# khanhha/multiview_motion_capture

Measured on AMD Instinct MI355X. Metric: frames/s (assoc+triangulate+IK) at C=5,P=4,J=25, higher is better.
Workload: dtype f64

## Files before the change

### include/mvmc.h

```cpp
#ifndef MVMC_H
#define MVMC_H

#include <stdint.h>

#ifdef __cplusplus
extern "C" {
#endif

#define MVMC_ABI_VERSION 6

enum {
    MVMC_OK = 0,
    MVMC_ERR_ARG = 1,
    MVMC_ERR_LAUNCH = 2,
    MVMC_ERR_UNSUPPORTED = 3
};

enum { MVMC_F32 = 0, MVMC_F64 = 1 };

#define MVMC_N_COCO 17
#define MVMC_N_SKEL 18
#define MVMC_N_SIDE 11
#define MVMC_N_PARAM 68
#define MVMC_MAX_NODES 80
// ... 160 lines not shown
    int32_t* out_meta;
    int32_t* out_n_tracks;
    double* out_info;
    int32_t* out_als_iters;
    uint32_t* flags;
    double* out_phase_cycles;
} mvmcChainBuffers;
int mvmc_chain_run(const mvmcSkeleton* skel_host, const mvmcChainBuffers* buffers, mvmcStream_t stream);

int mvmc_chain_run_rigs(const mvmcSkeleton* skel_host, const mvmcChainBuffers* buffers, const int32_t* rig_of_chain, int n_rigs,
                        mvmcStream_t stream);

int mvmc_chain_run_sessions(const mvmcSkeleton* skel_host, const mvmcChainBuffers* buffers, const int32_t* rig_of_chain, int n_rigs,
                            const uint8_t* active, mvmcStream_t stream);


int mvmc_body_observe(const double* kps17, const int32_t* counts, int n_frames, int n_views, int p_max, const double* Pmats,
                      int n_rigs, const int32_t* frame_of, const int32_t* rig_of, const double* joints, const int32_t* order,
                      const int32_t* grp_lo, const int32_t* grp_hi, const int32_t* rank, int n_problems, double min_score,
                      double max_dist, int32_t* choice, double* dist, int32_t* members, int32_t* n_views_out, mvmcStream_t stream);

#define MVMC_BODY_INFO_DOUBLES 16
#define MVMC_BODY_WORK_DOUBLES 270
int mvmc_body_lengths(const mvmcSkeleton* skel_host, const double* kps17, int n_views, int p_max, const double* Pmats,
                      const int32_t* rig_of, const int32_t* members, const double* params, const int32_t* id_lo, int n_ids,
                      double* lens, int32_t* free_mask, int fix_free, int max_iter, double mu0, double ftol, double xtol,
                      double* info, double* work, mvmcStream_t stream);

int mvmc_ik_solve_stages_rigs(const mvmcSkeleton* skel_host, const double* kps17, const double* Pmats, int n_rigs,
                              const int32_t* rig_of_problem, const int32_t* members, int n_problems, int v_max, int n_views,
// ... 115 lines not shown
```

### multiview_motion_capture_amd/_cabi.py

```python
from __future__ import annotations

import ctypes as C
import os

_LIB_PATH = os.environ.get("MVMC_LIB_PATH") or os.path.join(os.path.dirname(os.path.abspath(__file__)), "lib",
                                                           "libmvmc_hip.so")
_lib = None

MVMC_OK = 0
MVMC_ABI = 6
MVMC_F32, MVMC_F64 = 0, 1
N_PARAM = 68
MAX_NODES = 80
IK_SCRATCH_DOUBLES = 7680
IK_FD_WORK_DOUBLES = 40960
IK_STEP_OUT_DOUBLES = 240
BOUND_WORDS, ROW_WORDS = 56, 128
BODY_INFO_DOUBLES, BODY_WORK_DOUBLES = 16, 270
SMOOTH_K, SMOOTH_BLOCK_DOUBLES, SMOOTH_WORK_DOUBLES, SMOOTH_INFO_DOUBLES, SMOOTH_MAX_VIEWS = 39, 820, 3940, 32, 64
SMOOTH_COV_INFO_DOUBLES, SMOOTH_JOINTS = 8, 18
SMOOTH_WIN_MAX, SMOOTH_WIN_RING, SMOOTH_WIN_ITEM_INTS, SMOOTH_WIN_INFO_DOUBLES = 32, 66, 8, 16
RELINK_MAX_RECORDS, RELINK_REC_DOUBLES = 512, 120
RIG_TILE, RIG_MAX_CAMS, RIG_MAX_ITER, RIG_CAM_DOUBLES, RIG_INFO_DOUBLES = 64, 8, 24, 21, 64
LENS_DOUBLES, LENS_PINHOLE, LENS_BROWN, LENS_FISHEYE, LENS_MAX_ITER, LENS_FISHEYE_MAX_THETA = 16, 0, 1, 2, 12, 1.5
# ... 1 lines not shown
RIG_LOSS_NONE, RIG_LOSS_HUBER, RIG_LOSS_CAUCHY = 0, 1, 2
RIG_STOP = {0: "running", 1: "xtol", 2: "ftol", 3: "few_cameras", 4: "few_points", 5: "max_iter"}

SYMBOLS = (
    "mvmc_abi_version", "mvmc_status_string", "mvmc_als_seed_table", "mvmc_ingest", "mvmc_fmats",
    "mvmc_affinity", "mvmc_als_associate", "mvmc_closure_labels", "mvmc_cluster_members", "mvmc_dlt", "mvmc_triangulate_postopt", "mvmc_fk", "mvmc_ik_solve",
    "mvmc_fmats_from_projections", "mvmc_st_affinity", "mvmc_track_assign", "mvmc_track_commit", "mvmc_debug_eigh",
    "mvmc_debug_trstep", "mvmc_ik_solve_stages", "mvmc_chain_run", "mvmc_svt_associate", "mvmc_debug_ik_solve_fd", "mvmc_debug_ik_model_step", "mvmc_ingest_dlt", "mvmc_ingest_dlt_f32", "mvmc_pack_message_words", "mvmc_pack_work_words", "mvmc_stitch_work_words", "mvmc_pack_tracks", "mvmc_stitch_chains",
    "mvmc_chain_run_rigs", "mvmc_chain_run_sessions", "mvmc_body_observe", "mvmc_body_lengths", "mvmc_ik_solve_stages_rigs",
    "mvmc_smooth_blocks", "mvmc_smooth_step", "mvmc_smooth_cov", "mvmc_smooth_window_work_doubles", "mvmc_smooth_window", "mvmc_relink_work_words", "mvmc_relink",
    "mvmc_rig_part_doubles", "mvmc_rig_red_doubles", "mvmc_rig_start", "mvmc_rig_accumulate", "mvmc_rig_step",
    "mvmc_rig_accumulate_robust", "mvmc_rig_step_robust", "mvmc_rig_weights",
    "mvmc_rig_part_doubles_intr", "mvmc_rig_red_doubles_intr", "mvmc_rig_accumulate_intr", "mvmc_rig_step_intr",
    "mvmc_lens_undistort", "mvmc_lens_distort",
    "mvmc_pair_moments", "mvmc_pair_consensus", "mvmc_pair_refit",
)


class MvmcSkeleton(C.Structure):
    _fields_ = [("bone_dirs", (C.c_double * 3) * 18), ("parents", C.c_int32 * 18),
                ("side_map", C.c_int32 * 18), ("n_side", C.c_int32), ("ref_side_lens", C.c_double * 18)]


class MvmcChainBuffers(C.Structure):
    _INTS = ("n_chains", "chain_len", "n_views", "p_max", "t_max", "k_max", "v_max", "max_nfev_cold", "max_nfev_warm",
             "n_inits", "seed_len", "n_parts", "force_big", "hand_over")
    _PTRS = ("kps17", "counts", "Pmats", "Fmats", "F2", "seed_table", "params", "joints", "meta", "n_tracks", "next_id",
             "n_dead", "slot_src", "S_sp", "W_st", "group_counts", "labels_sp", "labels_st", "n_clusters_sp", "n_clusters_st",
             "iters_sp", "iters_st", "members", "n_members", "cold", "init", "status", "n_new", "ik_params", "ik_joints", "ik_info",
             "ik_scratch", "out_params", "out_joints", "out_meta", "out_n_tracks", "out_info", "out_als_iters", "flags", "out_phase_cycles")
    _fields_ = [(n, C.c_int32) for n in _INTS] + [(n, C.c_void_p) for n in _PTRS]


class MvmcError(RuntimeError):
    pass


def lib_path() -> str:
    return _LIB_PATH


def build_info():
    if os.environ.get("MVMC_LIB_PATH"):
        return None
    from . import _buildinfo
    return _buildinfo.read()
# ... 37 lines not shown
        "mvmc_dlt": [vp, vp, vp, i32, i32, i32, i32, i32, f64, vp, vp],
        "mvmc_ingest_dlt": [vp, i32, i32, i32, i32, i32, vp, f64, i32, f64, vp, vp, i32, i32, f64, vp, vp, vp],
        "mvmc_ingest_dlt_f32": [vp, i32, i32, i32, i32, vp, f64, i32, f64, vp, vp, i32, i32, f64, vp, vp, vp],
        "mvmc_triangulate_postopt": [vp, vp, vp, i32, i32, i32, i32, i32, vp, vp],
        "mvmc_fk": [SK, vp, i32, vp, vp, vp],
        "mvmc_ik_solve": [SK, vp, vp, vp, i32, i32, i32, i32, vp, vp, i32, i32, vp, vp, vp, vp, vp],
        "mvmc_fmats_from_projections": [vp, i32, vp, vp],
        "mvmc_st_affinity": [vp, vp, vp, vp, vp, vp, vp, i32, i32, i32, i32, f64, vp, vp, vp, vp],
        "mvmc_track_assign": [vp] * 8 + [i32] * 6 + [vp] * 7,
        "mvmc_track_commit": [vp] * 4 + [i32] * 4 + [vp] * 9,
        "mvmc_debug_eigh": [vp, vp, i32, i32, vp, vp, vp, vp, vp],
        "mvmc_debug_trstep": [vp, vp, i32, i32, i32, f64, f64, vp, vp, vp, vp],
        "mvmc_chain_run": [SK, C.POINTER(MvmcChainBuffers), vp],
        "mvmc_chain_run_rigs": [SK, C.POINTER(MvmcChainBuffers), vp, i32, vp],
        "mvmc_chain_run_sessions": [SK, C.POINTER(MvmcChainBuffers), vp, i32, vp, vp],
        "mvmc_ik_solve_stages": [SK, vp, vp, vp, vp, i32, i32, i32, i32, vp, i32, i32, vp, vp, vp, vp, vp],
        "mvmc_debug_ik_solve_fd": [SK, vp, vp, vp, i32, i32, i32, i32, vp, vp, i32, i32, i32, vp, vp, vp, vp, vp],
        "mvmc_debug_ik_model_step": [SK, vp, vp, vp, i32, i32, i32, i32, vp, i32, vp, vp, vp, vp, vp],
        "mvmc_pack_message_words": [i32, i32, i32, i32],
        "mvmc_pack_work_words": [i32, i32, i32],
        "mvmc_stitch_work_words": [i32, i32, i32],
        "mvmc_pack_tracks": [vp, vp, vp, vp, vp, i32, i32, i32, i32, i32, i32, i32, f64, vp, i32, vp, vp, vp],
        "mvmc_stitch_chains": [vp, C.c_longlong, i32, i32, i32, i32, i32, f64, i32, vp, vp, vp, vp, vp],
        "mvmc_body_observe": [vp, vp, i32, i32, i32, vp, i32, vp, vp, vp, vp, vp, vp, vp, i32, f64, f64, vp, vp, vp, vp, vp],
        "mvmc_body_lengths": [SK, vp, i32, i32, vp, vp, vp, vp, vp, i32, vp, vp, i32, i32, f64, f64, f64, vp, vp, vp],
        "mvmc_ik_solve_stages_rigs": [SK, vp, vp, i32, vp, vp, i32, i32, i32, i32, vp, i32, i32, vp, vp, vp, vp, vp],
        "mvmc_smooth_blocks": [SK, vp, i32, i32, vp, vp, vp, vp, vp, vp, i32, vp, vp],
        "mvmc_smooth_step": [SK, vp, vp, vp, vp, i32, i32, f64, f64, f64, f64, f64, f64, f64, i32, i32, vp, vp, vp, vp],
        "mvmc_smooth_cov": [SK, vp, vp, vp, i32, i32, f64, f64, f64, f64, f64, vp, i32, i32, vp, vp, vp, vp, vp, vp, vp, vp],
        "mvmc_smooth_window_work_doubles": [i32, i32],
# ... 46 lines not shown
```

### multiview_motion_capture_amd/csrc/mvmc_assoc.hip

```cpp
#if !defined(MVMC_DEVICE_ONLY) && !defined(MVMC_SMALL_WPS)
#define MVMC_SMALL_WPS 4
#define ALS4_WG_PER_CU 4
#endif
#include "mvmc_common.h"

namespace {

template <typename T>
__global__ void __launch_bounds__(256)
ingest_kernel(const T* __restrict__ kps, int C, int P, int J_in, const int32_t* __restrict__ counts_in,
              double min_score, int min_valid, double min_bb, double* __restrict__ kps17,
              int32_t* __restrict__ counts_out) {
    extern __shared__ double sm[];
    const int f = blockIdx.x;
    const int nq = C * P;
    double* pose = sm;
    int* keep = reinterpret_cast<int*>(sm + nq * 51);
    int* src_of = keep + nq;
    const T* src = kps + (size_t)f * nq * J_in * 3;
    for (int e = threadIdx.x; e < nq * 51; e += blockDim.x) {
        int q = e / 51, r = e - q * 51, j = r / 3, k = r - j * 3;
        int js = (J_in == 25) ? op25_to_coco17(j) : j;
        pose[e] = (double)src[(q * J_in + js) * 3 + k];
    }
    __syncthreads();
    for (int q = threadIdx.x; q < nq; q += blockDim.x) {
        int c = q / P, p = q - c * P;
        int cnt = counts_in ? counts_in[f * C + c] : P;
        int ok = 0;
        if (p < cnt) {
            int nv = 0;
            double x0 = 1e300, x1 = -1e300, y0 = 1e300, y1 = -1e300;
            for (int j = 0; j < 17; ++j) {
                const double* kp = pose + q * 51 + j * 3;
                if (kp[2] > min_score) {
                    ++nv;
                    x0 = fmin(x0, kp[0]); x1 = fmax(x1, kp[0]);
                    y0 = fmin(y0, kp[1]); y1 = fmax(y1, kp[1]);
                }
            }
            ok = (nv >= min_valid) && !((x1 - x0) < min_bb || (y1 - y0) < min_bb);
        }
        keep[q] = ok;
    }
    __syncthreads();
    for (int c = threadIdx.x; c < C; c += blockDim.x) {
        int k = 0;
        for (int p = 0; p < P; ++p)
            if (keep[c * P + p]) src_of[c * P + k++] = c * P + p;
        counts_out[f * C + c] = k;
        for (; k < P; ++k) src_of[c * P + k] = -1;
    }
    __syncthreads();
    double* out = kps17 + (size_t)f * nq * 51;
    for (int e = threadIdx.x; e < nq * 51; e += blockDim.x) {
        int d = e / 51, r = e - d * 51;
        int q = src_of[d];
        out[e] = q >= 0 ? pose[q * 51 + r] : 0.0;
    }
}

__device__ inline void m3mul(const double* A, const double* B, double* O) {
    for (int i = 0; i < 3; ++i)
        for (int j = 0; j < 3; ++j) {
            double s = 0;
            for (int k = 0; k < 3; ++k) s += A[i * 3 + k] * B[k * 3 + j];
            O[i * 3 + j] = s;
        }
}
__device__ inline void m3t(const double* A, double* O) {
    for (int i = 0; i < 3; ++i)
        for (int j = 0; j < 3; ++j) O[i * 3 + j] = A[j * 3 + i];
}
__device__ inline void m3v(const double* A, const double* x, double* o) {
// ... 1799 lines not shown
        }
    }
}

}

#ifndef MVMC_DEVICE_ONLY
extern "C" int mvmc_ingest(const void* kps, int dtype, int n_frames, int n_views, int p_max, int n_joints_in,
                           const int32_t* counts_in, double min_score, int min_valid, double min_bb_size,
                           double* kps17, int32_t* counts_out, mvmcStream_t stream) {
    if (!kps || !kps17 || !counts_out || n_frames < 0 || n_views <= 0 || p_max <= 0) return MVMC_ERR_ARG;
    if (n_joints_in != 25 && n_joints_in != 17) return MVMC_ERR_ARG;
    if (dtype != MVMC_F32 && dtype != MVMC_F64) return MVMC_ERR_ARG;
    if (n_frames == 0) return MVMC_OK;
    const int nq = n_views * p_max;
    size_t shm = (size_t)nq * 51 * sizeof(double) + (size_t)nq * 2 * sizeof(int);
    if (shm > 64 * 1024) return MVMC_ERR_UNSUPPORTED;
    hipStream_t s = (hipStream_t)stream;
    if (dtype == MVMC_F32)
        hipLaunchKernelGGL(ingest_kernel<float>, dim3(n_frames), dim3(256), shm, s, (const float*)kps, n_views, p_max,
                           n_joints_in, counts_in, min_score, min_valid, min_bb_size, kps17, counts_out);
    else
        hipLaunchKernelGGL(ingest_kernel<double>, dim3(n_frames), dim3(256), shm, s, (const double*)kps, n_views,
                           p_max, n_joints_in, counts_in, min_score, min_valid, min_bb_size, kps17, counts_out);
    MVMC_CHECK_LAUNCH();
    return MVMC_OK;
}

extern "C" int mvmc_fmats(const double* K, const double* Rt, int n_views, float* F, mvmcStream_t stream) {
    if (!K || !Rt || !F || n_views <= 0) return MVMC_ERR_ARG;
    int n = n_views * n_views;
// ... 84 lines not shown
```

### multiview_motion_capture_amd/csrc/mvmc_chain.hip

```cpp
#define MVMC_DEVICE_ONLY
#if !defined(MVMC_CHAIN_BIG_TU) && !defined(MVMC_SMALL_WPS)
#define MVMC_SMALL_WPS 4
#endif
#if !defined(MVMC_CHAIN_BIG_TU) && !defined(MVMC_PRIO_ALS) && !defined(MVMC_NO_PHASE_PRIO)
#define MVMC_PRIO_ALS 1
#define MVMC_PRIO_REST 1
#endif
#if defined(MVMC_WITH_IK_PAIR) && !defined(MVMC_CHAIN_BIG_TU) && !defined(MVMC_CHAIN_LAT_TU) && MVMC_SMALL_WPS >= 4
#define MVMC_IK_PAIR 1
#endif
#include <cstdlib>
#include "mvmc_common.h"
#include "mvmc_assoc.hip"
#include "mvmc_track.hip"
#include "mvmc_ik1.hip"

struct MvmcChainArgs {
    const double* kps17;
    const int32_t* counts;
    const double* Pm;
    const float* Fm;
    const double* F2;
    const double* seed;
    int seed_len;
// ... 26 lines not shown
    double* ik_scratch;
    double* out_params;
    double* out_joints;
    int32_t* out_meta;
    int32_t* out_n;
    double* out_info;
    int32_t* out_iters;
    double* out_cycles;
    int parts;
    int queue;
    unsigned* flags;
    int self_zero;
    const int32_t* rig;
    int n_rigs;
    const uint8_t* active;
};


namespace {

using ChainArgs = MvmcChainArgs;
using ChainArgsK = const __attribute__((address_space(4))) MvmcChainArgs;

struct ChainRig { const double* Pm; const float* Fm; const double* F2; bool ok; };
__device__ __forceinline__ ChainRig chain_rig(ChainArgsK& A, int b) {
    ChainRig g{A.Pm, A.Fm, A.F2, true};
    if (A.rig) {
        const int r = uni(mvmc_ld_i32(A.rig + b));
        g.ok = r >= 0 && r < A.n_rigs;
        if (g.ok && r > 0) {
// ... 60 lines not shown
        if (2 * 4 * P * 68 <= CH_KOFF_BIG && C * P <= 64) {
            st_pose_pairs_lines<ChainCfg<BIG>::NT>(arena.graph + CH_EOFF_BIG, arena.graph, kf, A.counts, f, F2, C, P, 0.1);
            Epre = arena.graph + CH_EOFF_BIG;
        }
    }
    st_affinity_wave<ChainCfg<BIG>::NT>(arena.graph, A.kps17, A.counts, 0, f, A.joints + (size_t)b * T * 54, A.n_tracks + b, Pm, F2, C, P,
                           T, 0.1, W, nullptr, A.gc + (size_t)b * (C + 1), Epre, C * P, kf);
    *done = 0;
}
__device__ __noinline__ void chain_pose_pairs(ChainArena<false>& arena_in, ChainArgsK& A, int f, const double* F2_in, int* done) {
    ChainArena<false>& arena = *uni(&arena_in);
    MVMC_ASSUME_LDS(&arena);
    st_pose_pairs(arena.graph + CH_EOFF, A.kps17, A.counts, f, uni(F2_in), A.C, A.P, 0.1);
    *done = 0;
}
template <bool BIG>
__device__ __noinline__ void chain_als_spatial(ChainArena<BIG>& arena_in, ChainArgsK& A, int b, int f, int* done) {
    ChainArena<BIG>& arena = *uni(&arena_in);
    MVMC_ASSUME_LDS(&arena);
    const int C = A.C, N = C * A.P;
    if constexpr (BIG)
        als5_graph<float, 72>(arena.als, 0, A.S_sp + (size_t)b * N * N, A.counts + (size_t)f * C, C, N, A.seed, A.seed_len,
                                          nullptr, nullptr, A.labels_sp + (size_t)b * N, A.ncl_sp + b, A.iters_sp + b);
    else
        als4_graph<float, 24>(arena.als_sp, 0, A.S_sp + (size_t)b * N * N, A.counts + (size_t)f * C, C, N, A.seed, A.seed_len, nullptr,
                              nullptr, A.labels_sp + (size_t)b * N, A.ncl_sp + b, A.iters_sp + b);
    *done = 0;
}
template <bool BIG>
__device__ __noinline__ void chain_als_temporal(ChainArena<BIG>& arena_in, ChainArgsK& A, int b, int* done) {
// ... 96 lines not shown
    }
    {
        static_assert(sizeof(Ik1Tables) % 4 == 0, "copied by words");
        typedef const __attribute__((address_space(4))) unsigned* KernargWords;
        KernargWords src = (KernargWords)__builtin_amdgcn_kernarg_segment_ptr();
        unsigned* dst = reinterpret_cast<unsigned*>(&tables);
        for (int i = tid; i < (int)(sizeof(Ik1Tables) / 4); i += ChainCfg<BIG>::NT) dst[i] = src[i];
    }
    int b, part;
    int done = 0;
    ChainRig rig{A.Pm, A.Fm, A.F2, true};
    if (!queue) {
        const int idx = by_ticket ? uni(s_nt) : (int)blockIdx.x;
        b = idx % A.n_chains; part = idx / A.n_chains;
        rig = chain_rig(A, b);
        if constexpr (!BIG) { if (part > 0 && rig.ok) chain_pose_pairs(arena, A, b * A.L + part * A.L / A.parts, rig.F2, &done); }
    }
    if (queue || part > 0) {
        if (tid == 0) {
            int task = queue ? (int)ticket : ((part << 20) | b);
            const bool must_wait = queue ? ticket >= (unsigned)A.n_chains : true;
            if (must_wait) {
                const unsigned* word = queue ? qwords + 2 + (ticket - (unsigned)A.n_chains) : A.flags + b;
                const unsigned need = queue ? 1u : (unsigned)part;
                const unsigned long long t0 = wall_clock64();
                bool abort = false;
                unsigned spins = 0, v;
                while ((v = __hip_atomic_load(word, __ATOMIC_RELAXED, __HIP_MEMORY_SCOPE_AGENT)) < need) {
                    __builtin_amdgcn_s_sleep(32);
                    if ((++spins & 1023u) != 0u) continue;
// ... 8 lines not shown
                asm volatile("s_waitcnt vmcnt(0)" ::: "memory");
                if (queue && !abort) task = (int)v - 1;
                if (abort) {
                    if (!queue) __hip_atomic_store(A.flags + b, (unsigned)(part + 1), __ATOMIC_RELAXED, __HIP_MEMORY_SCOPE_AGENT);
                    task = -1;
                }
            }
            s_task = task;
        }
        __syncthreads();
        const int task = uni(s_task);
        if (task < 0) return;
        b = task & 0xFFFFF; part = task >> 20;
        if (queue) {
            rig = chain_rig(A, b);
            if constexpr (!BIG) { if (part > 0 && rig.ok) chain_pose_pairs(arena, A, b * A.L + part * A.L / A.parts, rig.F2, &done); }
        }
    }
    if (A.active && uni((int)A.active[b]) == 0) return;
    const int T = A.T, NP = T + A.K;
    const int t_lo = part * A.L / A.parts;
    int t_hi = (part + 1) * A.L / A.parts;
    if (!rig.ok) {
        for (int t = t_lo + tid; t < t_hi; t += ChainCfg<BIG>::NT) A.out_n[b * A.L + t] = 0;
        if (tid == 0) atomicOr(A.flags + A.n_chains + 4 + b, 16u);
        t_hi = t_lo;
    }
    __syncthreads();
    long long cyc[6] = {0, 0, 0, 0, 0, 0}, t_prev = clock64();
    const long long t_start = t_prev;
    auto lap = [&](int k) { const long long now = clock64(); cyc[k] += now - t_prev; t_prev = now; };
    for (int t = t_lo; t < t_hi; ++t) {
        const int f = b * A.L + t;
        if (tid == 0) s_nt = mvmc_ld_i32(A.n_tracks + b);
        __syncthreads();
        const int nt = uni(s_nt);
#ifdef MVMC_PRIO_ALS
        if constexpr (!BIG) __builtin_amdgcn_s_setprio(MVMC_PRIO_ALS);
#endif
        if (nt <= 0) {
            chain_graph_spatial<BIG>(arena, A, b, f, rig.Fm, &done);
            __syncthreads();
            lap(0);
            chain_als_spatial<BIG>(arena, A, b, f, &done);
        } else {
            chain_graph_temporal<BIG>(arena, A, b, f, part > 0 && t == t_lo, rig.Pm, rig.F2, &done);
            __syncthreads();
            lap(0);
// ... 87 lines not shown
    MVMC_CHECK_LAUNCH();
    return MVMC_OK;
}
#else
extern "C" int mvmc_chain_run(const mvmcSkeleton* skel_host, const mvmcChainBuffers* buf, mvmcStream_t stream) {
    return mvmc_chain_run_rigs(skel_host, buf, nullptr, 1, stream);
}

extern "C" int mvmc_chain_run_rigs(const mvmcSkeleton* skel_host, const mvmcChainBuffers* buf, const int32_t* rig_of_chain, int n_rigs,
                                   mvmcStream_t stream) {
    return mvmc_chain_run_sessions(skel_host, buf, rig_of_chain, n_rigs, nullptr, stream);
}

extern "C" int mvmc_chain_run_sessions(const mvmcSkeleton* skel_host, const mvmcChainBuffers* buf, const int32_t* rig_of_chain, int n_rigs,
                                       const uint8_t* active, mvmcStream_t stream) {
    if (!skel_host || !buf) return MVMC_ERR_ARG;
    if (n_rigs < 1 || (!rig_of_chain && n_rigs != 1)) return MVMC_ERR_ARG;
    const mvmcChainBuffers& B = *buf;
    if (active && B.n_parts > 1) return MVMC_ERR_ARG;
    if (B.n_chains < 0 || B.chain_len <= 0 || B.n_views <= 0 || B.p_max <= 0 || B.t_max <= 0 || B.k_max <= 0 || B.v_max <= 0)
        return MVMC_ERR_ARG;
    if (B.max_nfev_cold < 1 || B.max_nfev_warm < 1) return MVMC_ERR_ARG;
    const int N = B.n_views * B.p_max, NS = B.t_max + N;
    if (B.n_views > 16 || 2 * B.p_max > 16) return MVMC_ERR_UNSUPPORTED;
    if (B.t_max + B.k_max > 64 || B.v_max > 64) return MVMC_ERR_UNSUPPORTED;
    const bool small = N <= ChainCfg<false>::N_MAX && NS <= ChainCfg<false>::NS_MAX && !B.force_big &&
                       2 * (B.t_max > B.p_max ? B.t_max : B.p_max) <= 16;
    const bool big = N <= ChainCfg<true>::N_MAX && NS <= ChainCfg<true>::NS_MAX && B.t_max <= 16;
    if (!small && !big) return MVMC_ERR_UNSUPPORTED;
    const void* need[] = {B.kps17, B.counts, B.Pmats, B.Fmats, B.F2, B.seed_table, B.params, B.joints, B.meta, B.n_tracks,
                          B.next_id, B.n_dead, B.slot_src, B.S_sp, B.W_st, B.group_counts, B.labels_sp, B.labels_st, B.n_clusters_sp,
// ... 15 lines not shown
    A.S_sp = B.S_sp; A.W_st = B.W_st; A.gc = B.group_counts; A.labels_sp = B.labels_sp; A.labels_st = B.labels_st;
    A.ncl_sp = B.n_clusters_sp; A.ncl_st = B.n_clusters_st; A.iters_sp = B.iters_sp; A.iters_st = B.iters_st;
    A.members = B.members; A.n_members = B.n_members; A.cold = B.cold; A.init = B.init; A.status = B.status;
    A.n_new = B.n_new; A.ik_params = B.ik_params; A.ik_joints = B.ik_joints; A.ik_info = B.ik_info; A.ik_scratch = B.ik_scratch;
    A.out_params = B.out_params; A.out_joints = B.out_joints; A.out_meta = B.out_meta; A.out_n = B.out_n_tracks;
    A.out_info = B.out_info; A.out_iters = B.out_als_iters; A.out_cycles = B.out_phase_cycles;
    A.parts = B.n_parts > 1 ? B.n_parts : 1;
    if (A.parts > 1 && B.chain_len % A.parts != 0) return MVMC_ERR_ARG;
    if (B.hand_over < 0 || B.hand_over > 2) return MVMC_ERR_ARG;
    A.queue = B.hand_over;
    if (B.n_chains >= (1 << 20) || A.parts >= (1 << 10)) return MVMC_ERR_UNSUPPORTED;
    A.flags = B.flags;
    A.self_zero = 0;
    A.rig = rig_of_chain; A.n_rigs = n_rigs;
    A.active = active;
    bool lat = false;
    if (small) {
        static const bool no_lat = getenv("MVMC_CHAIN_NO_LAT") && atoi(getenv("MVMC_CHAIN_NO_LAT")) != 0;
        int dev = 0, cus = 256;
        if (hipGetDevice(&dev) == hipSuccess) {
            int v = 0;
            if (hipDeviceGetAttribute(&v, hipDeviceAttributeMultiprocessorCount, dev) == hipSuccess && v > 0) cus = v;
        }
        lat = !no_lat && (long long)B.n_chains * A.parts <= 2LL * cus;
    }
    if (lat && B.n_chains == 1 && A.parts == 1)
        A.self_zero = 1;
    else if (hipMemsetAsync(B.flags, 0, sizeof(unsigned) * ((size_t)B.n_chains * (A.parts + 1) + 8), (hipStream_t)stream) != hipSuccess)
        return MVMC_ERR_LAUNCH;
    Ik1Tables tables_host;
// ... 16 lines not shown
```

### multiview_motion_capture_amd/pipeline.py

```python
from __future__ import annotations

from typing import Optional

import torch

from . import device as dev


class HotPath:
    def __init__(self, K, Rt, device="cuda:0", k_max: Optional[int] = None, v_max: Optional[int] = None):
        d = torch.device(device)
        self.device = d
        self.K = torch.as_tensor(K, dtype=torch.float64, device=d).contiguous()
        self.Rt = torch.as_tensor(Rt, dtype=torch.float64, device=d).contiguous()
        self.P = torch.bmm(self.K, self.Rt).contiguous()
        self.F = dev.fmats(self.K, self.Rt)
        self.skeleton = dev.make_skeleton()
        self.k_max = k_max
        self.v_max = v_max

    def associate(self, kps: torch.Tensor, counts: Optional[torch.Tensor] = None, want_mats=False):
        kps17, cnt = dev.ingest(kps, counts)
        P = kps17.shape[2]
        D, S = dev.affinity(kps17, cnt, self.F, want_D=want_mats)
        res = dev.als_associate(S, cnt, g_max=P, want_mats=want_mats)
        res.update(kps17=kps17, counts=cnt, D=D, S=S)
        return res

    def triangulate(self, assoc: dict):
        kps17, cnt = assoc["kps17"], assoc["counts"]
        C, P = kps17.shape[1], kps17.shape[2]
        k_max = self.k_max or max(1, (C * P) // 2)
        v_max = self.v_max or min(C * P, 64)
        mem, nm = dev.cluster_members(assoc["labels"], cnt, P, k_max, v_max)
# ... 19 lines not shown
```

### multiview_motion_capture_amd/tracker.py

```python
from __future__ import annotations

import ctypes
import os
from typing import Optional, Sequence

import numpy as np
import torch

from . import _cabi, device as dev
from .pipeline import HotPath

T_WIDE = 16


class ChainFlags:
    CLUSTER, TRACKS, GRAPH, IK_PAIR, RIG = 1, 2, 4, 8, 16
    REPAIRABLE = CLUSTER | TRACKS | GRAPH

    def __init__(self, words, n_chains: int):
        B = n_chains
        self.words, self.B, self._v0 = words, B, B + 4

    @staticmethod
    def length(n_chains: int, n_parts: int) -> int:
# ... 28 lines not shown
                                 (F.TRACKS, "more than t_max live tracklets")) if bits & bit]
        return ValueError(f"{who}: capacity exceeded (" + "; ".join(what) + f") in {n_void} chain(s): their results are void")
    return None


def _verdict_of(timeout, void: np.ndarray, who: str) -> Optional[Exception]:
    return void_verdict(int(timeout), int(np.bitwise_or.reduce(void)), int(np.count_nonzero(void)), who)


def _raise_if_void(timeout, void: np.ndarray, who: str) -> None:
    exc = _verdict_of(timeout, void, who)
    if exc is not None:
        raise exc


def chain_workspace(B: int, n_out: int, C: int, P: int, T: int, K: int, V: int, d, want_info: bool, flags) -> dict:
    N, NS, NP = C * P, T + C * P, T + K
    f64, i32 = torch.float64, torch.int32
    e = lambda shape, dt: torch.empty(shape, dtype=dt, device=d)
    z = lambda shape, dt: torch.zeros(shape, dtype=dt, device=d)
    return dict(
        seed_table=dev.als_seed_table(_cabi.MAX_NODES * _cabi.MAX_NODES, d),
        S_sp=e((B, N, N), torch.float32), W_st=e((B, NS, NS), f64), group_counts=e((B, C + 1), i32),
        labels_sp=e((B, N), i32), labels_st=e((B, NS), i32), n_clusters_sp=z((B,), i32), n_clusters_st=z((B,), i32),
        iters_sp=z((B,), i32), iters_st=z((B,), i32), members=e((B, NP, V), i32), n_members=z((B, NP), i32),
        cold=e((B, NP), torch.uint8), init=e((B, NP, 68), f64), status=e((B, T), i32), n_new=e((B,), i32),
        ik_params=e((B, NP, 68), f64), ik_joints=e((B, NP, 18, 3), f64), ik_info=e((B, NP, 8), f64),
        ik_scratch=dev.stream_buffer("chain_ik", B, (8, _cabi.IK_SCRATCH_DOUBLES), d),
        out_params=e((n_out, T, 68), f64), out_joints=e((n_out, T, 18, 3), f64), out_meta=e((n_out, T, 4), i32),
        out_n_tracks=e((n_out,), i32), out_info=e((n_out, NP, 8), f64) if want_info else None,
        out_als_iters=e((n_out,), i32) if want_info else None, out_phase_cycles=e((B, 8), f64) if want_info else None,
        flags=z((flags,), i32) if isinstance(flags, int) else flags)


def fill_chain_buffers(ints: dict, tensors: dict) -> "_cabi.MvmcChainBuffers":
    buf = _cabi.MvmcChainBuffers()
    odd = (set(ints) ^ set(buf._INTS)) | (set(tensors) ^ set(buf._PTRS))
    if odd:
        raise ValueError(f"a chain buffer is not named or not known: {sorted(odd)}")
    for name in buf._INTS:
        setattr(buf, name, int(ints[name]))
    for name in buf._PTRS:
        setattr(buf, name, None if tensors[name] is None else tensors[name].data_ptr())
    return buf


def launch_chain(skeleton, buf, d, rig_of_chain: Optional[torch.Tensor] = None, n_rigs: int = 1,
                 active: Optional[torch.Tensor] = None) -> None:
    lib, sk, bf = _cabi.load(), ctypes.byref(skeleton), ctypes.byref(buf)
    stream = ctypes.c_void_p(torch.cuda.current_stream(d).cuda_stream)
    rig = None if rig_of_chain is None else ctypes.c_void_p(rig_of_chain.data_ptr())
    if active is not None:
        _cabi.check(lib.mvmc_chain_run_sessions(sk, bf, rig, n_rigs, ctypes.c_void_p(active.data_ptr()), stream), "mvmc_chain_run_sessions")
    elif rig is not None:
        _cabi.check(lib.mvmc_chain_run_rigs(sk, bf, rig, n_rigs, stream), "mvmc_chain_run_rigs")
    else:
        _cabi.check(lib.mvmc_chain_run(sk, bf, stream), "mvmc_chain_run")


def default_caps(n_views: int, p_max: int):
    n = n_views * p_max
    return max(1, n // 2), min(n, 64)


class ChainTracker:
    def __init__(self, hp: HotPath, n_chains: int, p_max: int, t_max: int = 8, k_max: Optional[int] = None,
                 v_max: Optional[int] = None, nfev_cold=50, nfev_warm=5, rigs: Optional[Sequence[HotPath]] = None):
# ... 334 lines not shown
    if rigs is None and rig_of_chain is not None:
        raise ValueError("run_chains_fused: rig_of_chain needs rigs")
    roc = None if rigs is None else check_rig_of_chain(rig_of_chain, B, len(rigs))
    if parts is None:
        parts = L
    if parts > 1 and L % parts:
        raise ValueError("run_chains_fused: parts must divide the chain length")
    if hand_over is None:
        hand_over = "ticket"
    if hand_over not in ("static", "queue", "ticket"):
        raise ValueError("run_chains_fused: hand_over must be 'ticket', 'static' or 'queue'")
    T = t_max if t_max is not None else (T_WIDE if Cn * P > 40 else 8)
    k_def, v_def = default_caps(Cn, P)
    K = k_max or k_def
    V = v_max or v_def
    kps17, cnt = dev.ingest(kps, counts)
    d = kps.device
    if rigs is None:
        Pm, Fm, F2 = hp.P, hp.F, dev.fmats_from_projections(hp.P)
    else:
        Pm, Fm, F2 = stack_rigs(rigs, Cn)
    f64, i32 = torch.float64, torch.int32
    z = lambda shape, dt: torch.zeros(shape, dtype=dt, device=d)
    t = dict(chain_workspace(B, F, Cn, P, T, K, V, d, want_info, ChainFlags.length(B, parts)),
             kps17=kps17, counts=cnt, Pmats=Pm, Fmats=Fm, F2=F2,
             params=z((B, T, 68), f64), joints=z((B, T, 18, 3), f64), meta=z((B, T, 4), i32), n_tracks=z((B,), i32),
             next_id=z((B,), i32), n_dead=z((B,), i32), slot_src=torch.full((B, T), -1, dtype=i32, device=d))
    ints = dict(n_chains=B, chain_len=L, n_views=Cn, p_max=P, t_max=T, k_max=K, v_max=V, max_nfev_cold=nfev_cold,
                max_nfev_warm=nfev_warm, n_inits=3, seed_len=t["seed_table"].numel(), n_parts=parts, force_big=int(force_big),
                hand_over={"static": 0, "queue": 1, "ticket": 2}[hand_over])
    buf = fill_chain_buffers(ints, t)
    rig_dev = None if roc is None else torch.from_numpy(roc).to(d)
    if kernel_events is not None:
        k0, k1 = torch.cuda.Event(enable_timing=True), torch.cuda.Event(enable_timing=True)
        k0.record()
    launch_chain(hp.skeleton, buf, d, rig_dev, 1 if rigs is None else len(rigs))
    if kernel_events is not None:
        k1.record()
        kernel_events.append((k0, k1))
    fl = ChainFlags(t["flags"], B)
    res = dict(params=t["out_params"], joints=t["out_joints"], meta=t["out_meta"], n_tracks=t["out_n_tracks"],
               n_dead=t["n_dead"], next_id=t["next_id"], flags=t["flags"], void=fl.void, void_words=fl.status, n_chains=B,
               chain_len=L, _keepalive=dict(t, rig_of_chain=rig_dev))
    if rigs is not None:
        res["rigs"], res["rig_of_chain"] = list(rigs), roc
    if want_info:
        res["ik_info"] = t["out_info"].view(B, L, T + K, 8)
        res["als_iters"] = t["out_als_iters"].view(B, L)
        res["phase_cycles"] = t["out_phase_cycles"]
    return res

# ... 13 lines not shown
    if a.size and not np.issubdtype(a.dtype, np.integer):
        raise ValueError(f"rig_of_chain: integer indices, not {a.dtype}")
    if a.size and (a.min() < 0 or a.max() >= n_rigs):
        raise ValueError(f"rig_of_chain: indices in [{a.min()}, {a.max()}], the call has {n_rigs} rig(s)")
    return np.ascontiguousarray(a, dtype=np.int32)


def stack_rigs(rigs: Sequence[HotPath], n_views: int):
    if len(rigs) == 0:
        raise ValueError("rigs: at least one rig")
    for r, h in enumerate(rigs):
        if h.P.shape[0] != n_views:
            raise ValueError(f"rigs[{r}] has {h.P.shape[0]} cameras, the keypoints {n_views} views")
    Pm = torch.stack([h.P for h in rigs]).contiguous()
    Fm = torch.stack([h.F for h in rigs]).contiguous()
    F2 = torch.stack([dev.fmats_from_projections(h.P) for h in rigs]).contiguous()
    return Pm, Fm, F2


def check_chain_flags(res) -> None:
    if "flags" not in res:
        _raise_if_void(0, res["overflow"].cpu().numpy(), "run_chains")
        return
    fl = ChainFlags(res["flags"], res["n_chains"]).host()
    _raise_if_void(fl.timeout, fl.void, "mvmc_chain_run")


def repair_chains(hp: HotPath, kps: torch.Tensor, counts: Optional[torch.Tensor], res, nfev_cold=50, nfev_warm=5,
                  t_wide: int = T_WIDE, big_first: bool = True) -> int:
    B, L = res["n_chains"], res["chain_len"]
    fl = ChainFlags(res["flags"], B)
# ... 72 lines not shown
```

Baseline: 563,100.

## Fuse keypoint ingest and state init into the chain kernel

Moves the per-frame keypoint ingest (joint remap, validity filter, compaction) into the persistent chain kernel, which stages each frame in LDS scratch and publishes it with a release/acquire fence. Per-chain track state is now zeroed on the device, so the separate ingest launch and the host-side torch.zeros/full allocations are replaced by empty tensors. It also caches F2 per hot path so it is no longer recomputed on every call. This cuts launch and memset overhead at the cost of extra in-kernel syncs and ingest work on the critical path.

New measurement: 564,400 (median of 6 runs). Within noise of the previous version (+0.2%).

```diff
diff --git a/include/mvmc.h b/include/mvmc.h
--- a/include/mvmc.h
+++ b/include/mvmc.h
@@ -198,6 +198,20 @@
 int mvmc_chain_run_sessions(const mvmcSkeleton* skel_host, const mvmcChainBuffers* buffers, const int32_t* rig_of_chain, int n_rigs,
                             const uint8_t* active, mvmcStream_t stream);
 
+typedef struct mvmcChainFront {
+    const void* kps_raw;
+    int32_t kps_dtype;
+    int32_t n_joints_in;
+    const int32_t* counts_in;
+    double ingest_min_score;
+    int32_t min_valid;
+    double min_bb_size;
+    int32_t fresh_state;
+} mvmcChainFront;
+
+int mvmc_chain_run_front(const mvmcSkeleton* skel_host, const mvmcChainBuffers* buffers, const mvmcChainFront* front,
+                         const int32_t* rig_of_chain, int n_rigs, const uint8_t* active, mvmcStream_t stream);
+
 
 int mvmc_body_observe(const double* kps17, const int32_t* counts, int n_frames, int n_views, int p_max, const double* Pmats,
                       int n_rigs, const int32_t* frame_of, const int32_t* rig_of, const double* joints, const int32_t* order,
diff --git a/multiview_motion_capture_amd/_cabi.py b/multiview_motion_capture_amd/_cabi.py
--- a/multiview_motion_capture_amd/_cabi.py
+++ b/multiview_motion_capture_amd/_cabi.py
@@ -39,6 +39,7 @@
     "mvmc_rig_part_doubles_intr", "mvmc_rig_red_doubles_intr", "mvmc_rig_accumulate_intr", "mvmc_rig_step_intr",
     "mvmc_lens_undistort", "mvmc_lens_distort",
     "mvmc_pair_moments", "mvmc_pair_consensus", "mvmc_pair_refit",
+    "mvmc_chain_run_front",
 )
 
 
@@ -55,6 +56,11 @@
              "iters_sp", "iters_st", "members", "n_members", "cold", "init", "status", "n_new", "ik_params", "ik_joints", "ik_info",
              "ik_scratch", "out_params", "out_joints", "out_meta", "out_n_tracks", "out_info", "out_als_iters", "flags", "out_phase_cycles")
     _fields_ = [(n, C.c_int32) for n in _INTS] + [(n, C.c_void_p) for n in _PTRS]
+
+
+class MvmcChainFront(C.Structure):
+    _fields_ = [("kps_raw", C.c_void_p), ("kps_dtype", C.c_int32), ("n_joints_in", C.c_int32), ("counts_in", C.c_void_p),
+                ("ingest_min_score", C.c_double), ("min_valid", C.c_int32), ("min_bb_size", C.c_double), ("fresh_state", C.c_int32)]
 
 
 class MvmcError(RuntimeError):
@@ -122,6 +128,7 @@
         "mvmc_chain_run": [SK, C.POINTER(MvmcChainBuffers), vp],
         "mvmc_chain_run_rigs": [SK, C.POINTER(MvmcChainBuffers), vp, i32, vp],
         "mvmc_chain_run_sessions": [SK, C.POINTER(MvmcChainBuffers), vp, i32, vp, vp],
+        "mvmc_chain_run_front": [SK, C.POINTER(MvmcChainBuffers), C.POINTER(MvmcChainFront), vp, i32, vp, vp],
         "mvmc_ik_solve_stages": [SK, vp, vp, vp, vp, i32, i32, i32, i32, vp, i32, i32, vp, vp, vp, vp, vp],
         "mvmc_debug_ik_solve_fd": [SK, vp, vp, vp, i32, i32, i32, i32, vp, vp, i32, i32, i32, vp, vp, vp, vp, vp],
         "mvmc_debug_ik_model_step": [SK, vp, vp, vp, i32, i32, i32, i32, vp, i32, vp, vp, vp, vp, vp],
diff --git a/multiview_motion_capture_amd/csrc/mvmc_assoc.hip b/multiview_motion_capture_amd/csrc/mvmc_assoc.hip
--- a/multiview_motion_capture_amd/csrc/mvmc_assoc.hip
+++ b/multiview_motion_capture_amd/csrc/mvmc_assoc.hip
@@ -3,6 +3,7 @@
 #define ALS4_WG_PER_CU 4
 #endif
 #include "mvmc_common.h"
+#include "mvmc_ingest.h"
 
 namespace {
 
@@ -12,52 +13,7 @@
               double min_score, int min_valid, double min_bb, double* __restrict__ kps17,
               int32_t* __restrict__ counts_out) {
     extern __shared__ double sm[];
-    const int f = blockIdx.x;
-    const int nq = C * P;
-    double* pose = sm;
-    int* keep = reinterpret_cast<int*>(sm + nq * 51);
-    int* src_of = keep + nq;
-    const T* src = kps + (size_t)f * nq * J_in * 3;
-    for (int e = threadIdx.x; e < nq * 51; e += blockDim.x) {
-        int q = e / 51, r = e - q * 51, j = r / 3, k = r - j * 3;
-        int js = (J_in == 25) ? op25_to_coco17(j) : j;
-        pose[e] = (double)src[(q * J_in + js) * 3 + k];
-    }
-    __syncthreads();
-    for (int q = threadIdx.x; q < nq; q += blockDim.x) {
-        int c = q / P, p = q - c * P;
-        int cnt = counts_in ? counts_in[f * C + c] : P;
-        int ok = 0;
-        if (p < cnt) {
-            int nv = 0;
-            double x0 = 1e300, x1 = -1e300, y0 = 1e300, y1 = -1e300;
-            for (int j = 0; j < 17; ++j) {
-                const double* kp = pose + q * 51 + j * 3;
-                if (kp[2] > min_score) {
-                    ++nv;
-                    x0 = fmin(x0, kp[0]); x1 = fmax(x1, kp[0]);
-                    y0 = fmin(y0, kp[1]); y1 = fmax(y1, kp[1]);
-                }
-            }
-            ok = (nv >= min_valid) && !((x1 - x0) < min_bb || (y1 - y0) < min_bb);
-        }
-        keep[q] = ok;
-    }
-    __syncthreads();
-    for (int c = threadIdx.x; c < C; c += blockDim.x) {
-        int k = 0;
-        for (int p = 0; p < P; ++p)
-            if (keep[c * P + p]) src_of[c * P + k++] = c * P + p;
-        counts_out[f * C + c] = k;
-        for (; k < P; ++k) src_of[c * P + k] = -1;
-    }
-    __syncthreads();
-    double* out = kps17 + (size_t)f * nq * 51;
-    for (int e = threadIdx.x; e < nq * 51; e += blockDim.x) {
-        int d = e / 51, r = e - d * 51;
-        int q = src_of[d];
-        out[e] = q >= 0 ? pose[q * 51 + r] : 0.0;
-    }
+    ingest_frame<T>(sm, threadIdx.x, blockDim.x, blockIdx.x, kps, C, P, J_in, counts_in, min_score, min_valid, min_bb, kps17, counts_out);
 }
 
 __device__ inline void m3mul(const double* A, const double* B, double* O) {
@@ -1887,7 +1843,7 @@
     if (dtype != MVMC_F32 && dtype != MVMC_F64) return MVMC_ERR_ARG;
     if (n_frames == 0) return MVMC_OK;
     const int nq = n_views * p_max;
-    size_t shm = (size_t)nq * 51 * sizeof(double) + (size_t)nq * 2 * sizeof(int);
+    size_t shm = (size_t)ingest_stage_doubles(nq) * sizeof(double);
     if (shm > 64 * 1024) return MVMC_ERR_UNSUPPORTED;
     hipStream_t s = (hipStream_t)stream;
     if (dtype == MVMC_F32)
diff --git a/multiview_motion_capture_amd/csrc/mvmc_chain.hip b/multiview_motion_capture_amd/csrc/mvmc_chain.hip
--- a/multiview_motion_capture_amd/csrc/mvmc_chain.hip
+++ b/multiview_motion_capture_amd/csrc/mvmc_chain.hip
@@ -64,6 +64,11 @@
     const int32_t* rig;
     int n_rigs;
     const uint8_t* active;
+    const void* kps_raw;
+    const int32_t* counts_in;
+    double in_min_score, in_min_bb;
+    int kps_f32, J_in, in_min_valid;
+    int fresh_state;
 };
 
 
@@ -154,6 +159,43 @@
     st_pose_pairs(arena.graph + CH_EOFF, A.kps17, A.counts, f, uni(F2_in), A.C, A.P, 0.1);
     *done = 0;
 }
+__device__ __forceinline__ void chain_publish_rows() {
+    asm volatile("s_waitcnt vmcnt(0)" ::: "memory");
+    __syncthreads();
+    if ((threadIdx.x >> 6) == 0) {
+        __builtin_amdgcn_fence(__ATOMIC_RELEASE, "agent");
+        asm volatile("s_waitcnt vmcnt(0)" ::: "memory");
+        __builtin_amdgcn_fence(__ATOMIC_ACQUIRE, "agent");
+    }
+    __syncthreads();
+}
+template <bool BIG>
+__device__ __noinline__ void chain_ingest(ChainArena<BIG>& arena_in, ChainArgsK& A, int f, int* done) {
+    ChainArena<BIG>& arena = *uni(&arena_in);
+    MVMC_ASSUME_LDS(&arena);
+    static_assert(ingest_stage_doubles(ChainCfg<BIG>::N_MAX) <= (int)(sizeof(ChainArena<BIG>::graph) / sizeof(double)), "the staging fits the graph scratch");
+    constexpr int NT = ChainCfg<BIG>::NT;
+    double* kps17 = const_cast<double*>(A.kps17);
+    int32_t* counts = const_cast<int32_t*>(A.counts);
+    if (A.kps_f32)
+        ingest_frame<float>(arena.graph, threadIdx.x, NT, f, static_cast<const float*>(A.kps_raw), A.C, A.P, A.J_in, A.counts_in, A.in_min_score,
+                            A.in_min_valid, A.in_min_bb, kps17, counts);
+    else
+        ingest_frame<double>(arena.graph, threadIdx.x, NT, f, static_cast<const double*>(A.kps_raw), A.C, A.P, A.J_in, A.counts_in, A.in_min_score,
+                             A.in_min_valid, A.in_min_bb, kps17, counts);
+    chain_publish_rows();
+    *done = 0;
+}
+__device__ __noinline__ void chain_fresh_state(ChainArgsK& A, int b, int nthreads, int* done) {
+    const int tid = threadIdx.x, T = A.T;
+    for (int e = tid; e < T * 68; e += nthreads) A.params[(size_t)b * T * 68 + e] = 0.0;
+    for (int e = tid; e < T * 54; e += nthreads) A.joints[(size_t)b * T * 54 + e] = 0.0;
+    for (int e = tid; e < T * 4; e += nthreads) A.meta[(size_t)b * T * 4 + e] = 0;
+    for (int e = tid; e < T; e += nthreads) A.slot_src[(size_t)b * T + e] = -1;
+    if (tid == 0) { A.n_tracks[b] = 0; A.next_id[b] = 0; A.n_dead[b] = 0; }
+    chain_publish_rows();
+    *done = 0;
+}
 template <bool BIG>
 __device__ __noinline__ void chain_als_spatial(ChainArena<BIG>& arena_in, ChainArgsK& A, int b, int f, int* done) {
     ChainArena<BIG>& arena = *uni(&arena_in);
@@ -280,6 +322,7 @@
         const int idx = by_ticket ? uni(s_nt) : (int)blockIdx.x;
         b = idx % A.n_chains; part = idx / A.n_chains;
         rig = chain_rig(A, b);
+        if (A.kps_raw && rig.ok && !(A.active && uni((int)A.active[b]) == 0)) chain_ingest<BIG>(arena, A, b * A.L + part * A.L / A.parts, &done);
         if constexpr (!BIG) { if (part > 0 && rig.ok) chain_pose_pairs(arena, A, b * A.L + part * A.L / A.parts, rig.F2, &done); }
     }
     if (queue || part > 0) {
@@ -318,10 +361,12 @@
         b = task & 0xFFFFF; part = task >> 20;
         if (queue) {
             rig = chain_rig(A, b);
+            if (A.kps_raw && rig.ok) chain_ingest<BIG>(arena, A, b * A.L + part * A.L / A.parts, &done);
             if constexpr (!BIG) { if (part > 0 && rig.ok) chain_pose_pairs(arena, A, b * A.L + part * A.L / A.parts, rig.F2, &done); }
         }
     }
     if (A.active && uni((int)A.active[b]) == 0) return;
+    if (A.fresh_state && part == 0) chain_fresh_state(A, b, ChainCfg<BIG>::NT, &done);
     const int T = A.T, NP = T + A.K;
     const int t_lo = part * A.L / A.parts;
     int t_hi = (part + 1) * A.L / A.parts;
@@ -336,6 +381,7 @@
     auto lap = [&](int k) { const long long now = clock64(); cyc[k] += now - t_prev; t_prev = now; };
     for (int t = t_lo; t < t_hi; ++t) {
         const int f = b * A.L + t;
+        if (A.kps_raw && t > t_lo) chain_ingest<BIG>(arena, A, f, &done);
         if (tid == 0) s_nt = mvmc_ld_i32(A.n_tracks + b);
         __syncthreads();
         const int nt = uni(s_nt);
@@ -453,7 +499,17 @@
 
 extern "C" int mvmc_chain_run_sessions(const mvmcSkeleton* skel_host, const mvmcChainBuffers* buf, const int32_t* rig_of_chain, int n_rigs,
                                        const uint8_t* active, mvmcStream_t stream) {
+    return mvmc_chain_run_front(skel_host, buf, nullptr, rig_of_chain, n_rigs, active, stream);
+}
+
+extern "C" int mvmc_chain_run_front(const mvmcSkeleton* skel_host, const mvmcChainBuffers* buf, const mvmcChainFront* front,
+                                    const int32_t* rig_of_chain, int n_rigs, const uint8_t* active, mvmcStream_t stream) {
     if (!skel_host || !buf) return MVMC_ERR_ARG;
+    if (front) {
+        if (!front->kps_raw || (front->kps_dtype != MVMC_F32 && front->kps_dtype != MVMC_F64)) return MVMC_ERR_ARG;
+        if (front->n_joints_in != 25 && front->n_joints_in != 17) return MVMC_ERR_ARG;
+        if (front->fresh_state && active) return MVMC_ERR_ARG;
+    }
     if (n_rigs < 1 || (!rig_of_chain && n_rigs != 1)) return MVMC_ERR_ARG;
     const mvmcChainBuffers& B = *buf;
     if (active && B.n_parts > 1) return MVMC_ERR_ARG;
@@ -499,6 +555,12 @@
     A.self_zero = 0;
     A.rig = rig_of_chain; A.n_rigs = n_rigs;
     A.active = active;
+    A.kps_raw = front ? front->kps_raw : nullptr;
+    A.counts_in = front ? front->counts_in : nullptr;
+    A.in_min_score = front ? front->ingest_min_score : 0.0; A.in_min_bb = front ? front->min_bb_size : 0.0;
+    A.kps_f32 = front && front->kps_dtype == MVMC_F32; A.J_in = front ? front->n_joints_in : 0;
+    A.in_min_valid = front ? front->min_valid : 0;
+    A.fresh_state = front && front->fresh_state;
     bool lat = false;
     if (small) {
         static const bool no_lat = getenv("MVMC_CHAIN_NO_LAT") && atoi(getenv("MVMC_CHAIN_NO_LAT")) != 0;
diff --git a/multiview_motion_capture_amd/csrc/mvmc_ingest.h b/multiview_motion_capture_amd/csrc/mvmc_ingest.h
--- /dev/null
+++ b/multiview_motion_capture_amd/csrc/mvmc_ingest.h
@@ -0,0 +1,55 @@
+#pragma once
+#include "mvmc_common.h"
+
+__host__ __device__ constexpr int ingest_stage_doubles(int nq) { return nq * 52; }
+
+template <typename T>
+__device__ __forceinline__ void ingest_frame(double* sm, int tid, int nt, int f, const T* __restrict__ kps, int C, int P, int J_in,
+                                             const int32_t* __restrict__ counts_in, double min_score, int min_valid, double min_bb,
+                                             double* __restrict__ kps17, int32_t* __restrict__ counts_out) {
+    const int nq = C * P;
+    double* pose = sm;
+    int* keep = reinterpret_cast<int*>(sm + nq * 51);
+    int* src_of = keep + nq;
+    const T* src = kps + (size_t)f * nq * J_in * 3;
+    for (int e = tid; e < nq * 51; e += nt) {
+        int q = e / 51, r = e - q * 51, j = r / 3, k = r - j * 3;
+        int js = (J_in == 25) ? op25_to_coco17(j) : j;
+        pose[e] = (double)src[(q * J_in + js) * 3 + k];
+    }
+    __syncthreads();
+    for (int q = tid; q < nq; q += nt) {
+        int c = q / P, p = q - c * P;
+        int cnt = counts_in ? counts_in[f * C + c] : P;
+        int ok = 0;
+        if (p < cnt) {
+            int nv = 0;
+            double x0 = 1e300, x1 = -1e300, y0 = 1e300, y1 = -1e300;
+            for (int j = 0; j < 17; ++j) {
+                const double* kp = pose + q * 51 + j * 3;
+                if (kp[2] > min_score) {
+                    ++nv;
+                    x0 = fmin(x0, kp[0]); x1 = fmax(x1, kp[0]);
+                    y0 = fmin(y0, kp[1]); y1 = fmax(y1, kp[1]);
+                }
+            }
+            ok = (nv >= min_valid) && !((x1 - x0) < min_bb || (y1 - y0) < min_bb);
+        }
+        keep[q] = ok;
+    }
+    __syncthreads();
+    for (int c = tid; c < C; c += nt) {
+        int k = 0;
+        for (int p = 0; p < P; ++p)
+            if (keep[c * P + p]) src_of[c * P + k++] = c * P + p;
+        counts_out[f * C + c] = k;
+        for (; k < P; ++k) src_of[c * P + k] = -1;
+    }
+    __syncthreads();
+    double* out = kps17 + (size_t)f * nq * 51;
+    for (int e = tid; e < nq * 51; e += nt) {
+        int d = e / 51, r = e - d * 51;
+        int q = src_of[d];
+        out[e] = q >= 0 ? pose[q * 51 + r] : 0.0;
+    }
+}
diff --git a/multiview_motion_capture_amd/pipeline.py b/multiview_motion_capture_amd/pipeline.py
--- a/multiview_motion_capture_amd/pipeline.py
+++ b/multiview_motion_capture_amd/pipeline.py
@@ -18,6 +18,13 @@
         self.skeleton = dev.make_skeleton()
         self.k_max = k_max
         self.v_max = v_max
+        self._F2 = None
+
+    @property
+    def F2(self) -> torch.Tensor:
+        if self._F2 is None:
+            self._F2 = dev.fmats_from_projections(self.P)
+        return self._F2
 
     def associate(self, kps: torch.Tensor, counts: Optional[torch.Tensor] = None, want_mats=False):
         kps17, cnt = dev.ingest(kps, counts)
diff --git a/multiview_motion_capture_amd/tracker.py b/multiview_motion_capture_amd/tracker.py
--- a/multiview_motion_capture_amd/tracker.py
+++ b/multiview_motion_capture_amd/tracker.py
@@ -66,11 +66,11 @@
         raise exc
 
 
-def chain_workspace(B: int, n_out: int, C: int, P: int, T: int, K: int, V: int, d, want_info: bool, flags) -> dict:
+def chain_workspace(B: int, n_out: int, C: int, P: int, T: int, K: int, V: int, d, want_info: bool, flags, zeroed: bool = True) -> dict:
     N, NS, NP = C * P, T + C * P, T + K
     f64, i32 = torch.float64, torch.int32
     e = lambda shape, dt: torch.empty(shape, dtype=dt, device=d)
-    z = lambda shape, dt: torch.zeros(shape, dtype=dt, device=d)
+    z = (lambda shape, dt: torch.zeros(shape, dtype=dt, device=d)) if zeroed else e
     return dict(
         seed_table=dev.als_seed_table(_cabi.MAX_NODES * _cabi.MAX_NODES, d),
         S_sp=e((B, N, N), torch.float32), W_st=e((B, NS, NS), f64), group_counts=e((B, C + 1), i32),
@@ -97,12 +97,32 @@
     return buf
 
 
+def chain_front(kps: torch.Tensor, counts: Optional[torch.Tensor], fresh_state: bool, min_score=0.01, min_valid=4,
+                min_bb=5.0) -> "_cabi.MvmcChainFront":
+    if kps.dtype not in (torch.float32, torch.float64):
+        raise ValueError("chain_front: kps must be float32 or float64")
+    if kps.dim() != 5 or kps.shape[3] not in (17, 25) or kps.shape[4] != 3 or not kps.is_contiguous():
+        raise ValueError(f"chain_front: expected contiguous (F,C,P,25|17,3), got {tuple(kps.shape)}")
+    if counts is not None and (counts.dtype != torch.int32 or tuple(counts.shape) != tuple(kps.shape[:2]) or not counts.is_contiguous()
+                               or counts.device != kps.device):
+        raise ValueError(f"chain_front: counts must be contiguous int32 {tuple(kps.shape[:2])} on {kps.device}")
+    fr = _cabi.MvmcChainFront()
+    fr.kps_raw, fr.counts_in = kps.data_ptr(), None if counts is None else counts.data_ptr()
+    fr.kps_dtype = _cabi.MVMC_F32 if kps.dtype == torch.float32 else _cabi.MVMC_F64
+    fr.n_joints_in, fr.ingest_min_score, fr.min_valid, fr.min_bb_size = int(kps.shape[3]), float(min_score), int(min_valid), float(min_bb)
+    fr.fresh_state = int(bool(fresh_state))
+    return fr
+
+
 def launch_chain(skeleton, buf, d, rig_of_chain: Optional[torch.Tensor] = None, n_rigs: int = 1,
-                 active: Optional[torch.Tensor] = None) -> None:
+                 active: Optional[torch.Tensor] = None, front: Optional["_cabi.MvmcChainFront"] = None) -> None:
     lib, sk, bf = _cabi.load(), ctypes.byref(skeleton), ctypes.byref(buf)
     stream = ctypes.c_void_p(torch.cuda.current_stream(d).cuda_stream)
     rig = None if rig_of_chain is None else ctypes.c_void_p(rig_of_chain.data_ptr())
-    if active is not None:
+    if front is not None:
+        act = None if active is None else ctypes.c_void_p(active.data_ptr())
+        _cabi.check(lib.mvmc_chain_run_front(sk, bf, ctypes.byref(front), rig, n_rigs, act, stream), "mvmc_chain_run_front")
+    elif active is not None:
         _cabi.check(lib.mvmc_chain_run_sessions(sk, bf, rig, n_rigs, ctypes.c_void_p(active.data_ptr()), stream), "mvmc_chain_run_sessions")
     elif rig is not None:
         _cabi.check(lib.mvmc_chain_run_rigs(sk, bf, rig, n_rigs, stream), "mvmc_chain_run_rigs")
@@ -467,18 +487,25 @@
     k_def, v_def = default_caps(Cn, P)
     K = k_max or k_def
     V = v_max or v_def
-    kps17, cnt = dev.ingest(kps, counts)
     d = kps.device
+    f64, i32 = torch.float64, torch.int32
+    n_flags = ChainFlags.length(B, parts)
     if rigs is None:
-        Pm, Fm, F2 = hp.P, hp.F, dev.fmats_from_projections(hp.P)
+        front = chain_front(kps, counts, fresh_state=True)
+        e = lambda shape, dt: torch.empty(shape, dtype=dt, device=d)
+        t = dict(chain_workspace(B, F, Cn, P, T, K, V, d, want_info, e((n_flags,), i32) if B else n_flags, zeroed=False),
+                 kps17=e((F, Cn, P, 17, 3), f64), counts=e((F, Cn), i32), Pmats=hp.P, Fmats=hp.F, F2=hp.F2,
+                 params=e((B, T, 68), f64), joints=e((B, T, 18, 3), f64), meta=e((B, T, 4), i32), n_tracks=e((B,), i32),
+                 next_id=e((B,), i32), n_dead=e((B,), i32), slot_src=e((B, T), i32))
     else:
+        front = None
+        kps17, cnt = dev.ingest(kps, counts)
         Pm, Fm, F2 = stack_rigs(rigs, Cn)
-    f64, i32 = torch.float64, torch.int32
-    z = lambda shape, dt: torch.zeros(shape, dtype=dt, device=d)
-    t = dict(chain_workspace(B, F, Cn, P, T, K, V, d, want_info, ChainFlags.length(B, parts)),
-             kps17=kps17, counts=cnt, Pmats=Pm, Fmats=Fm, F2=F2,
-             params=z((B, T, 68), f64), joints=z((B, T, 18, 3), f64), meta=z((B, T, 4), i32), n_tracks=z((B,), i32),
-             next_id=z((B,), i32), n_dead=z((B,), i32), slot_src=torch.full((B, T), -1, dtype=i32, device=d))
+        z = lambda shape, dt: torch.zeros(shape, dtype=dt, device=d)
+        t = dict(chain_workspace(B, F, Cn, P, T, K, V, d, want_info, n_flags),
+                 kps17=kps17, counts=cnt, Pmats=Pm, Fmats=Fm, F2=F2,
+                 params=z((B, T, 68), f64), joints=z((B, T, 18, 3), f64), meta=z((B, T, 4), i32), n_tracks=z((B,), i32),
+                 next_id=z((B,), i32), n_dead=z((B,), i32), slot_src=torch.full((B, T), -1, dtype=i32, device=d))
     ints = dict(n_chains=B, chain_len=L, n_views=Cn, p_max=P, t_max=T, k_max=K, v_max=V, max_nfev_cold=nfev_cold,
                 max_nfev_warm=nfev_warm, n_inits=3, seed_len=t["seed_table"].numel(), n_parts=parts, force_big=int(force_big),
                 hand_over={"static": 0, "queue": 1, "ticket": 2}[hand_over])
@@ -487,7 +514,7 @@
     if kernel_events is not None:
         k0, k1 = torch.cuda.Event(enable_timing=True), torch.cuda.Event(enable_timing=True)
         k0.record()
-    launch_chain(hp.skeleton, buf, d, rig_dev, 1 if rigs is None else len(rigs))
+    launch_chain(hp.skeleton, buf, d, rig_dev, 1 if rigs is None else len(rigs), front=front)
     if kernel_events is not None:
         k1.record()
         kernel_events.append((k0, k1))
@@ -531,7 +558,7 @@
             raise ValueError(f"rigs[{r}] has {h.P.shape[0]} cameras, the keypoints {n_views} views")
     Pm = torch.stack([h.P for h in rigs]).contiguous()
     Fm = torch.stack([h.F for h in rigs]).contiguous()
-    F2 = torch.stack([dev.fmats_from_projections(h.P) for h in rigs]).contiguous()
+    F2 = torch.stack([h.F2 for h in rigs]).contiguous()
     return Pm, Fm, F2
 
 
```
